# KDL-umass/CausalGPSLC.jl

Hardware: AMD Instinct MI355X
Metric: posterior samples/sec (kernel+chol+predict) at N=4096; SATE rel-err vs CPU (higher is better)
Workload: dtype f64; 1 GPU; Synthetic N=4096 D=8 nU=2, unit A (Gram build + potrf + alpha + MeanITE + SATE mean/var), L=1 level(s), 1024 posterior samples per GPU per step; levels=1, mean_ite=True

## Files before the change

### causalgpslc.jl_amd/csrc/k_gram.hip

```cpp
#include "gpslc_internal.h"
#include "gp_math.h"
#include <type_traits>

template <typename RT, int BIN, int FT>
__global__ __launch_bounds__(256) void gram_kernel(GramArgs g) {
    extern __shared__ __attribute__((aligned(16))) double sm[];
    const int F = FT > 0 ? FT : g.nU + g.nX;
    double* red = sm;
    double* etab = red + 4 * GP_TS * 2;
    RT* fr = reinterpret_cast<RT*>(etab + GP_EXP_TAB_DOUBLES);
    RT* fc = fr + F * GP_TS;
    RT* tr = fc + F * GP_TS;
    RT* tc = tr + GP_TS;

    const int tid = threadIdx.x;
    const int b = blockIdx.y;
    const long long s = g.s0 + b;
#ifdef GPSLC_DIAG
    const unsigned long long dt0 = g.dbg ? __builtin_amdgcn_s_memtime() : 0;
    const unsigned long long dr0 = g.dbg ? __builtin_amdgcn_s_memrealtime() : 0;
#endif
    int ti, tj;
    tri_decode(blockIdx.x, ti, tj);
    const int n = g.n;
    const int gi0 = ti * GP_TS, gj0 = tj * GP_TS;

    if (FT > 0) {
        constexpr int NIT = (FT * GP_TS + 255) / 256;
        constexpr bool CENTRE = std::is_same<RT, float>::value;
        double lv[NIT > 0 ? NIT : 1], av[NIT > 0 ? NIT : 1], cv[NIT > 0 ? NIT : 1];
        [[maybe_unused]] double x0[CENTRE && NIT > 0 ? NIT : 1];
#pragma unroll
        for (int k = 0; k < NIT; ++k) {
            const int idx = tid + 256 * k;
            const int f = min(idx >> 7, FT - 1), r = idx & 127;
            const double* src = g.column(s, f);
            lv[k] = g.lengthscale(s, f);
            av[k] = src[min(gi0 + r, n - 1)];
            cv[k] = src[min(gj0 + r, n - 1)];
            if constexpr (CENTRE) x0[k] = src[0];
        }
#pragma unroll
        for (int k = 0; k < NIT; ++k) {
            const int idx = tid + 256 * k;
            if (idx < FT * GP_TS) {
                const int f = idx >> 7, r = idx & 127;
                const double il = 1.0 / lv[k];
                if constexpr (CENTRE) { av[k] -= x0[k]; cv[k] -= x0[k]; }
                fr[f * GP_TS + r] = (RT)((gi0 + r < n) ? av[k] * il : 0.0);
                fc[f * GP_TS + r] = (RT)((gj0 + r < n) ? cv[k] * il : 0.0);
            }
        }
    } else {
        stage_scaled_features<GP_TS>(g, s, F, F, gi0, fr);
        stage_scaled_features<GP_TS>(g, s, F, F, gj0, fc);
    }
    if (tid < GP_TS) {
        tr[tid] = (RT)((gi0 + tid < n) ? centred_value<RT>(g.T, gi0 + tid) : 0.0);
        tc[tid] = (RT)((gj0 + tid < n) ? centred_value<RT>(g.T, gj0 + tid) : 0.0);
    }
    gp_exp_tab_stage(etab, tid);
    __syncthreads();
#ifdef GPSLC_DIAG
    const unsigned long long dt1 = g.dbg ? __builtin_amdgcn_s_memtime() : 0;
#endif

    const double ys = g.p.yScale[s];
    const double yn = g.p.yNoise[s];
    const double tl = g.p.tyLS[s];
    const RT wt = (RT)(1.0 / (tl * tl));
    const RT ew = RbfMath<RT>::exp_neg_t(-wt, etab);
    const int ty = tid & 15, tx = tid >> 4;

    RT tra[8];
#pragma unroll
    for (int p = 0; p < 8; ++p) tra[p] = tr[ty + 16 * p];

    double* tile = tref_tile(g.M, b, ti, tj);
    const int Np = g.nt * GP_TS;
    double* partB = g.part + ((long long)b * 2 + 0) * g.nt * Np;
    double* partK = g.part + ((long long)b * 2 + 1) * g.nt * Np;
    double rsB[8], rsK[8];
#pragma unroll
    for (int p = 0; p < 8; ++p) { rsB[p] = 0.0; rsK[p] = 0.0; }

    auto columns = [&](auto fast_tag) {
        constexpr bool FAST = decltype(fast_tag)::value;
#pragma unroll 1
        for (int q = 0; q < 8; ++q) {
            const int cq = 8 * tx + q;
            const int gj = gj0 + cq;
            RT lux[8];
#pragma unroll
            for (int p = 0; p < 8; ++p) lux[p] = (RT)0;
#pragma unroll 2
            for (int f = 0; f < (FT > 0 ? FT : F); ++f) {
                const RT c = fc[f * GP_TS + cq];
#pragma unroll
                for (int p = 0; p < 8; ++p) {
                    const RT d = fr[f * GP_TS + ty + 16 * p] - c;
                    lux[p] = fma(d, d, lux[p]);
                }
            }
            const RT tcq = tc[cq];
            double csB = 0.0, csK = 0.0;
#pragma unroll
            for (int p = 0; p < 8; ++p) {
                const int rp = ty + 16 * p;
                const int gi = gi0 + rp;
                const RT dt = tra[p] - tcq;
                const RT Bq = (RT)ys * RbfMath<RT>::exp_neg_t(-lux[p], etab);
                const RT Eq = BIN ? (dt == (RT)0 ? (RT)1 : ew) : RbfMath<RT>::exp_neg_t(-((dt * dt) * wt), etab);
                double Bv, Kv, Av;
                if (FAST) {
                    Bv = (double)Bq; Kv = (double)Bq * (double)Eq; Av = Kv;
                } else {
                    const bool inside = (gi < n) && (gj < n);
                    Bv = inside ? (double)Bq : 0.0;
                    Kv = inside ? (double)Bq * (double)Eq : 0.0;
                    Av = (gi == gj) ? (inside ? Kv + yn : 1.0) : Kv;
                }
                __builtin_nontemporal_store(Av, &tile[cq * GP_TS + rp]);
                rsB[p] += Bv; rsK[p] += Kv;
                csB += Bv; csK += Kv;
            }
            if (g.with_sums) {
#pragma unroll
                for (int o = 1; o <= 8; o <<= 1) { csB += __shfl_xor(csB, o, 64); csK += __shfl_xor(csK, o, 64); }
                if (ty == 0) {
                    partB[(long long)ti * Np + gj] = csB;
                    partK[(long long)ti * Np + gj] = csK;
                }
            }
        }
    };
    if (ti != tj && gi0 + GP_TS <= n && gj0 + GP_TS <= n) columns(std::true_type{});
    else columns(std::false_type{});
#ifdef GPSLC_DIAG
    if (g.dbg) {
        const unsigned long long dt2 = __builtin_amdgcn_s_memtime();
        asm volatile("s_waitcnt vmcnt(0)" ::: "memory");
        if (tid == 0) {
            unsigned long long* d = g.dbg + 8 * ((size_t)blockIdx.y * gridDim.x + blockIdx.x);
            d[0] = dt0; d[1] = dt1; d[2] = dt2; d[3] = __builtin_amdgcn_s_memtime();
            d[4] = dr0; d[5] = __builtin_amdgcn_s_memrealtime();
        }
    }
#endif
    if (!g.with_sums || ti == tj) return;

    const int wave = tid >> 6, lane = tid & 63;
    __syncthreads();
#pragma unroll
    for (int p = 0; p < 8; ++p) {
        double vb = rsB[p], vk = rsK[p];
        vb += __shfl_xor(vb, 16, 64); vk += __shfl_xor(vk, 16, 64);
        vb += __shfl_xor(vb, 32, 64); vk += __shfl_xor(vk, 32, 64);
        if (lane < 16) {
            red[(wave * GP_TS + ty + 16 * p) * 2 + 0] = vb;
            red[(wave * GP_TS + ty + 16 * p) * 2 + 1] = vk;
        }
    }
    __syncthreads();
    if (tid < GP_TS) {
        const double vb = (red[(0 * GP_TS + tid) * 2] + red[(1 * GP_TS + tid) * 2]) +
                          (red[(2 * GP_TS + tid) * 2] + red[(3 * GP_TS + tid) * 2]);
        const double vk = (red[(0 * GP_TS + tid) * 2 + 1] + red[(1 * GP_TS + tid) * 2 + 1]) +
                          (red[(2 * GP_TS + tid) * 2 + 1] + red[(3 * GP_TS + tid) * 2 + 1]);
        partB[(long long)tj * Np + gi0 + tid] = vb;
        partK[(long long)tj * Np + gi0 + tid] = vk;
    }
}

#define GRAM_LDS_BYTES(F, RTS) (4 * GP_TS * 2 * 8 + GP_EXP_TAB_DOUBLES * 8 + (2 * (F) * GP_TS + 2 * GP_TS) * (RTS))

template <typename RT, int BIN, int FT>
static void launch_gram_t(const GramArgs& g, int nbatch, hipStream_t st) {
    const int F = g.nU + g.nX;
    static DeviceOnce attr_set;
    lds_opt_in(attr_set, (const void*)gram_kernel<RT, BIN, FT>, GRAM_LDS_BYTES(MAXF, (int)sizeof(RT)));
    const int nlow = g.nt * (g.nt + 1) / 2;
    hipLaunchKernelGGL((gram_kernel<RT, BIN, FT>), dim3(nlow, nbatch), dim3(256), GRAM_LDS_BYTES(F, (int)sizeof(RT)), st, g);
}
template <typename RT, int BIN>
static void launch_gram_b(const GramArgs& g, int nbatch, hipStream_t st) {
    switch (g.nU + g.nX) {
        case 4: launch_gram_t<RT, BIN, 4>(g, nbatch, st); break;
        case 5: launch_gram_t<RT, BIN, 5>(g, nbatch, st); break;
        case 6: launch_gram_t<RT, BIN, 6>(g, nbatch, st); break;
        case 8: launch_gram_t<RT, BIN, 8>(g, nbatch, st); break;
        case 10: launch_gram_t<RT, BIN, 10>(g, nbatch, st); break;
        case 12: launch_gram_t<RT, BIN, 12>(g, nbatch, st); break;
        case 20: launch_gram_t<RT, BIN, 20>(g, nbatch, st); break;
        default: launch_gram_t<RT, BIN, 0>(g, nbatch, st); break;
    }
}
void launch_gram(const GramArgs& g, int nbatch, hipStream_t st) {
    if (g.f32) { if (g.binary_t) launch_gram_b<float, 1>(g, nbatch, st); else launch_gram_b<float, 0>(g, nbatch, st); }
    else { if (g.binary_t) launch_gram_b<double, 1>(g, nbatch, st); else launch_gram_b<double, 0>(g, nbatch, st); }
}

template <int FORM>
__global__ __launch_bounds__(256) void rhs_prepare_kernel(RhsArgs a) {
    using LF = LevelForm<FORM>;
    __shared__ double red[4];
    const int tid = threadIdx.x;
    const int b = blockIdx.x;
    const long long s = a.s0 + b;
    const int Np = a.nt * GP_TS;
    const double* partB = a.part + ((long long)b * 2 + 0) * a.nt * Np;
    const double* partK = a.part + ((long long)b * 2 + 1) * a.nt * Np;
    double* bs = a.bsum + (long long)b * Np;
    double* ks = a.ksum + (long long)b * Np;
    double tb = 0.0, tk = 0.0;
    for (int j = tid; j < Np; j += 256) {
        double vb = 0.0, vk = 0.0;
        for (int slot = 0; slot < a.nt; ++slot) {
            vb += partB[(long long)slot * Np + j];
            vk += partK[(long long)slot * Np + j];
        }
        bs[j] = vb; ks[j] = vk;
        tb += vb; tk += vk;
    }
    const double btot = block_sum_256(tb, red);
    const double ktot = block_sum_256(tk, red);
    const double tl = a.tyLS[s];
    const double wt = 1.0 / (tl * tl);
    const int L = a.lv.L;
    if constexpr (!LF::factual) {
        for (int l = tid; l < L; l += 256) {
            const double rho = LF::paired ? gp_rho(a.lv.doT[l], a.lv.base[l], wt) : 0.0;
            a.sumdelta[(long long)b * L + l] = LF::prior(rho, wt) * btot;
        }
        return;
    }
    for (int l = 0; l < L; ++l) {
        const double dot = a.lv.doT[l];
        double acc = 0.0;
        for (int j = tid; j < Np; j += 256) {
            const double r = gp_rho(j < a.n ? a.T[j] : 0.0, dot, wt);
            acc += r * bs[j];
        }
        const double rb = block_sum_256(acc, red);
        if (tid == 0) a.sumdelta[(long long)b * L + l] = (ktot - 2.0 * rb) + btot;
    }
}

template <int FORM>
__device__ __forceinline__ double rhs_level_value(const RhsArgs& a, int l, int gj, double wt, const double* bs, const double* ks) {
    using LF = LevelForm<FORM>;
    const double r = gp_rho(a.T[gj], a.lv.doT[l], wt);
    const double rb = LF::paired ? gp_rho(a.T[gj], a.lv.base[l], wt) : 0.0;
    const double x = LF::cross(a.T[gj] - a.lv.doT[l], r, rb, wt);
    if constexpr (LF::factual) return x * bs[gj] - ks[gj];
    else return x * bs[gj];
}
template <int FORM>
__global__ __launch_bounds__(256) void rhs_tiles_kernel(RhsArgs a) {
    const int tid = threadIdx.x;
    const int j = blockIdx.x, au = blockIdx.y, b = blockIdx.z;
    if (j > a.nt + au) return;
    const long long s = a.s0 + b;
    double* tile = tref_tile(a.M, b, a.nt + au, j);
    if (j >= a.nt) {
        if (a.live_rows > 0) return;
        for (int idx = tid; idx < GP_TSQ; idx += 256) tile[idx] = 0.0;
        return;
    }
    const int Np = a.nt * GP_TS;
    const int L = a.lv.L, R = L * a.G;
    const double tl = a.tyLS[s];
    const double wt = 1.0 / (tl * tl);
    const int sh = a.live_rows > 0 ? 5 : 7;
    for (int idx = tid; idx < (GP_TS << sh); idx += 256) {
        const int c = idx >> sh, q = idx & ((1 << sh) - 1);
        const int gq = au * GP_TS + q;
        const int gj = j * GP_TS + c;
        double v = 0.0;
        if (gj < a.n) {
            if (gq == 0) v = a.Y[s * a.y_sstride + gj];
            else if (gq <= R) {
                const int g = a.G > 1 ? (gq - 1) / L : 0, l = gq - 1 - L * g;
                const long long o = ((long long)b * a.G + g) * Np;
                v = rhs_level_value<FORM>(a, l, gj, wt, a.bw + o, a.kw + o);
            }
        }
        tile[c * GP_TS + q] = v;
    }
}

template <int FORM>
__global__ __launch_bounds__(256) void rhs_w_prepare_kernel(RhsArgs a) {
    using LF = LevelForm<FORM>;
    __shared__ double red[4];
    const int tid = threadIdx.x;
    const int qq = blockIdx.x, b = blockIdx.y;
    const int L = a.lv.L, l = qq % L, g = qq / L;
    const long long s = a.s0 + b;
    const int Np = a.nt * GP_TS;
    const double* bs = a.bw + ((long long)b * a.G + g) * Np;
    const double* ks = a.kw + ((long long)b * a.G + g) * Np;
    const double tl = a.tyLS[s];
    const double wt = 1.0 / (tl * tl);
    const double dot = a.lv.doT[l];
    double acc = 0.0, ww = 0.0;
    for (int j = tid; j < a.n; j += 256) {
        const double w = a.W[(long long)j * a.G + g];
        ww = fma(w, w, ww);
        if constexpr (!LF::factual) {
            acc += w * bs[j];
        } else {
            const double r = gp_rho(a.T[j], dot, wt);
            acc += w * ((ks[j] - 2.0 * r * bs[j]) + bs[j]);
        }
    }
    const double tot = block_sum_256(acc, red);
    if (l == 0) {
        const double w2 = block_sum_256(ww, red);
        if (tid == 0) a.wnorm2[(long long)b * a.G + g] = w2;
    }
    if (tid != 0) return;
    const double rho = LF::paired ? gp_rho(dot, a.lv.base[l], wt) : 0.0;
    if constexpr (LF::factual) a.sumdelta[(long long)b * L * a.G + qq] = tot;
    else a.sumdelta[(long long)b * L * a.G + qq] = LF::prior(rho, wt) * tot;
}

template <int FORM>
static void launch_rhs_t(const RhsArgs& r, int nbatch, hipStream_t st, bool sums_given) {
    if (r.W && !sums_given) hipLaunchKernelGGL(rhs_w_prepare_kernel<FORM>, dim3(r.lv.L * r.G, nbatch), dim3(256), 0, st, r);
    else if (r.with_sums && !sums_given) hipLaunchKernelGGL(rhs_prepare_kernel<FORM>, dim3(nbatch), dim3(256), 0, st, r);
    hipLaunchKernelGGL(rhs_tiles_kernel<FORM>, dim3(r.nt + r.naug, r.naug, nbatch), dim3(256), 0, st, r);
}
void launch_rhs(const RhsArgs& r, int nbatch, hipStream_t st, bool sums_given) {
    dispatch_form(r.lv.form, [&](auto form) { launch_rhs_t<decltype(form)::value>(r, nbatch, st, sums_given); });
}

__global__ __launch_bounds__(256) void epilogue_kernel(EpiArgs e) {
    __shared__ double red[4];
    const int tid = threadIdx.x;
    const int b = blockIdx.x;
    const long long s = e.s0 + b;
    double acc = 0.0;
    for (int i = tid; i < e.n; i += 256) {
        const int k = i >> 7, c = i & 127;
        const double* dt = tref_tile(e.M, b, k, k);
        acc += log(dt[c * GP_TS + c]);
    }
    const double ld = 2.0 * block_sum_256(acc, red);
    const double nn = (double)e.n;
    auto put_level = [&](int l, double zw, double ww) {
        const double sd = e.sumdelta[(long long)b * e.L + l];
        if (e.wnorm2) {
            if (e.meanSATE) e.meanSATE[s + e.S * l] = zw;
            if (e.varSATE) e.varSATE[s + e.S * l] = (sd - ww) + e.pred_noise * e.wnorm2[(long long)b * (e.L / e.wL) + l / e.wL];
            return;
        }
        if (e.meanSATE) e.meanSATE[s + e.S * l] = zw / nn;
        if (e.varSATE) e.varSATE[s + e.S * l] = ((sd - ww) + nn * e.pred_noise) / (nn * nn);
    };
    if (e.from_rows) {
        const int lane = tid & 63, wave = tid >> 6;
        const int ncol = e.nt * GP_TS;
        const int nq = (e.meanSATE || e.varSATE) ? e.L : 0;
        if (tid == 0 && e.logdet) e.logdet[s] = ld;
        auto put = [&](int q, double zw, double ww) {
            if (q == 0) { if (e.quad) e.quad[s] = ww; return; }
            put_level(q - 1, zw, ww);
        };
        if (nq >= 16) {
            for (int qb = 16 * wave; qb <= nq; qb += 64) {
                double zw[16], ww[16];
#pragma unroll
                for (int j = 0; j < 16; ++j) { zw[j] = 0.0; ww[j] = 0.0; }
                for (int i = lane; i < ncol; i += 64) {
                    const double* col = tref_tile(e.M, b, e.nt, i >> 7) + (long long)(i & 127) * GP_TS;
                    const double z = col[0];
#pragma unroll
                    for (int j = 0; j < 16; ++j) {
                        const double w = col[qb + j];
                        zw[j] = fma(z, w, zw[j]);
                        ww[j] = fma(w, w, ww[j]);
                    }
                }
#pragma unroll
                for (int j = 0; j < 16; ++j) {
                    double a = zw[j], c = ww[j];
#pragma unroll
                    for (int o = 32; o >= 1; o >>= 1) { a += __shfl_xor(a, o, 64); c += __shfl_xor(c, o, 64); }
                    if (lane == 0 && qb + j <= nq) put(qb + j, a, c);
                }
            }
            return;
        }
        for (int q = wave; q <= nq; q += 4) {
            double zw = 0.0, ww = 0.0;
            for (int i = lane; i < ncol; i += 64) {
                const double* col = tref_tile(e.M, b, e.nt, i >> 7) + (long long)(i & 127) * GP_TS;
                const double z = col[0], w = col[q];
                zw = fma(z, w, zw);
                ww = fma(w, w, ww);
            }
#pragma unroll
            for (int o = 32; o >= 1; o >>= 1) { zw += __shfl_xor(zw, o, 64); ww += __shfl_xor(ww, o, 64); }
            if (lane == 0) put(q, zw, ww);
        }
        return;
    }
    const double* g00 = tref_tile(e.M, b, e.nt, e.nt);
    if (tid == 0) {
        if (e.logdet) e.logdet[s] = ld;
        if (e.quad) e.quad[s] = -g00[0];
    }
    if (e.meanSATE == nullptr && e.varSATE == nullptr) return;
    for (int l = tid; l < e.L; l += 256) {
        const int q = 1 + l, au = q >> 7, qq = q & 127;
        const double wz = -tref_tile(e.M, b, e.nt + au, e.nt)[0 * GP_TS + qq];
        const double ww = -tref_tile(e.M, b, e.nt + au, e.nt + au)[qq * GP_TS + qq];
        put_level(l, wz, ww);
    }
}

void launch_epilogue(const EpiArgs& e, int nbatch, hipStream_t st) {
    hipLaunchKernelGGL(epilogue_kernel, dim3(nbatch), dim3(256), 0, st, e);
}

__global__ __launch_bounds__(256) void rbf_log_kernel(const double* X1, const double* X2, long long n,
                                                      int d, const double* ls, int ls_len, double* out) {
    const long long i = (long long)blockIdx.x * 16 + (threadIdx.x & 15);
    const long long ip = (long long)blockIdx.y * 16 + (threadIdx.x >> 4);
    if (i >= n || ip >= n) return;
    double acc = 0.0;
    for (int k = 0; k < d; ++k) {
        const double l = ls[ls_len == 1 ? 0 : k];
        const double df = X1[i + n * k] - X2[ip + n * k];
        acc += (df * df) / (l * l);
    }
    out[i + n * ip] = -acc;
}

void launch_rbf_log(const double* X1, const double* X2, long long n, int d, const double* ls,
                    int ls_len, double* out, hipStream_t st) {
    dim3 grid((unsigned)((n + 15) / 16), (unsigned)((n + 15) / 16));
    hipLaunchKernelGGL(rbf_log_kernel, grid, dim3(256), 0, st, X1, X2, n, d, ls, ls_len, out);
}

__global__ __launch_bounds__(256) void process_cov_kernel(const double* in, long long n, double scale,
                                                          double noise, double* out) {
    const long long idx = (long long)blockIdx.x * 256 + threadIdx.x;
    if (idx >= n * n) return;
    const long long i = idx % n, j = idx / n;
    double v = exp(in[idx]) * scale;
    if (i == j) v += noise;
    out[idx] = v;
}

void launch_process_cov(const double* in, long long n, double scale, double noise, double* out,
                        hipStream_t st) {
    const long long tot = n * n;
    hipLaunchKernelGGL(process_cov_kernel, dim3((unsigned)((tot + 255) / 256)), dim3(256), 0, st, in, n,
                       scale, noise, out);
}

__global__ __launch_bounds__(256) void dense_load_kernel(DenseLoadArgs a) {
    int ti, tj;
    tri_decode(blockIdx.x, ti, tj);
    double* tile = tref_tile(a.M, 0, ti, tj);
    for (int idx = threadIdx.x; idx < GP_TSQ; idx += 256) {
        const int c = idx >> 7, r = idx & 127;
        const long long gi = (long long)ti * GP_TS + r, gj = (long long)tj * GP_TS + c;
        double v;
        if (gi < a.n && gj < a.n) v = a.cov[gi + (long long)a.n * gj];
        else v = (gi == gj) ? 1.0 : 0.0;
        tile[idx] = v;
    }
}
void launch_dense_load(const DenseLoadArgs& a, hipStream_t st) {
    hipLaunchKernelGGL(dense_load_kernel, dim3(a.nt * (a.nt + 1) / 2), dim3(256), 0, st, a);
}

__global__ __launch_bounds__(256) void rows_rhs_kernel(RowsRhsArgs a) {
    const int j = blockIdx.x, au = blockIdx.y;
    if (a.rect ? (j >= a.nt) : (j > a.nt + au)) return;
    double* tile = tref_tile(a.M, 0, a.row0 + au, j);
    for (int idx = threadIdx.x; idx < GP_TSQ; idx += 256) {
        const int c = idx >> 7, q = idx & 127;
        const long long gq = (long long)au * GP_TS + q, gj = (long long)j * GP_TS + c;
        double v = 0.0;
        if (j < a.nt && gq < a.S && gj < a.n) v = a.x[gj + (long long)a.n * gq];
        tile[idx] = v;
    }
}
void launch_rows_rhs(const RowsRhsArgs& a, hipStream_t st) {
    hipLaunchKernelGGL(rows_rhs_kernel, dim3(a.nt + a.naug, a.naug), dim3(256), 0, st, a);
}

__global__ __launch_bounds__(256) void quad_rows_kernel(QuadRowsArgs a) {
    __shared__ double red[4];
    const int tid = threadIdx.x;
    double acc = 0.0;
    for (int i = tid; i < a.n; i += 256) {
        const double* dt = tref_tile(a.M, 0, i >> 7, i >> 7);
        acc += log(dt[(i & 127) * GP_TS + (i & 127)]);
    }
    const double ld = 2.0 * block_sum_256(acc, red);
    if (tid == 0) a.logdet[0] = ld;
    for (long long q = tid; q < a.S; q += 256) {
        const int au = (int)(q >> 7), qq = (int)(q & 127);
        a.quad[q] = -tref_tile(a.M, 0, a.nt + au, a.nt + au)[qq * GP_TS + qq];
    }
}
__global__ __launch_bounds__(128) void row_norms_kernel(RowNormArgs a) {
    const int au = blockIdx.x, q = threadIdx.x;
    double acc = 0.0;
    for (int j = 0; j < a.nt; ++j) {
        const double* t = tref_tile(a.W, 0, au, j);
        for (int c = 0; c < GP_TS; ++c) {
            const double v = t[c * GP_TS + q];
            acc = fma(v, v, acc);
        }
    }
    const long long gq = (long long)au * GP_TS + q;
    if (gq < a.S) a.quad[gq] = acc;
}
void launch_row_norms(const RowNormArgs& a, hipStream_t st) {
    hipLaunchKernelGGL(row_norms_kernel, dim3(a.naug), dim3(128), 0, st, a);
}

void launch_quad_rows(const QuadRowsArgs& a, hipStream_t st) {
    hipLaunchKernelGGL(quad_rows_kernel, dim3(1), dim3(256), 0, st, a);
}
```

### causalgpslc.jl_amd/csrc/k_solve.hip

```cpp
#include "gpslc_internal.h"
#include "gp_math.h"
#include "back_block.h"
#include "pair_mfma.h"
#include <stdexcept>

__global__ __launch_bounds__(256) void backsolve_alpha_kernel(BackArgs a, int i, double* alpha) {
    __shared__ double zi[GP_TS];
    const int tid = threadIdx.x, lane = tid & 63, wave = tid >> 6;
    const long long b = blockIdx.x;
    const int Np = a.nt * GP_TS;
    if (tid < GP_TS) zi[tid] = a.zwork[b * Np + i * GP_TS + tid];
    __syncthreads();
    const double* invt = a.inv + b * a.inv_bstride + (long long)i * GP_TSQ;
    double o32[32];
    tile_tv32(invt, zi, wave, lane, o32);
    if (lane == 0) {
#pragma unroll
        for (int cc = 0; cc < 32; ++cc) alpha[b * Np + i * GP_TS + wave * 32 + cc] = o32[cc];
    }
}
__global__ __launch_bounds__(256) void backsolve_update_kernel(BackArgs a, int i, const double* alpha) {
    __shared__ double ai[GP_TS];
    const int tid = threadIdx.x, lane = tid & 63, wave = tid >> 6;
    const int k = blockIdx.x;
    const long long b = blockIdx.y;
    const int Np = a.nt * GP_TS;
    if (tid < GP_TS) ai[tid] = alpha[b * Np + i * GP_TS + tid];
    __syncthreads();
    double o32[32];
    tile_tv32(tref_tile(a.M, b, i, k), ai, wave, lane, o32);
    double* z = a.zwork + b * Np;
    if (lane == 0) {
#pragma unroll
        for (int cc = 0; cc < 32; ++cc) z[k * GP_TS + wave * 32 + cc] -= o32[cc];
    }
}

__global__ __launch_bounds__(128) void extract_z_kernel(BackArgs a) {
    const int j = blockIdx.x;
    const long long b = blockIdx.y;
    const double* t = tref_tile(a.M, b, a.nt, j);
    a.zwork[b * a.nt * GP_TS + j * GP_TS + threadIdx.x] = t[threadIdx.x * GP_TS + 0];
}

void launch_backsolve(const BackArgs& a, int nbatch, hipStream_t st) {
    double* alpha = a.zwork + (long long)nbatch * a.nt * GP_TS;
    hipLaunchKernelGGL(extract_z_kernel, dim3(a.nt, nbatch), dim3(128), 0, st, a);
    for (int i = a.nt - 1; i >= 0; --i) {
        hipLaunchKernelGGL(backsolve_alpha_kernel, dim3(nbatch), dim3(256), 0, st, a, i, alpha);
        if (i > 0) hipLaunchKernelGGL(backsolve_update_kernel, dim3(i, nbatch), dim3(256), 0, st, a, i, alpha);
    }
}

template <int FREG, int LCT, typename RT, int RB, int FORM = FORM_ORDINARY>
__global__ __launch_bounds__(256) void ite_mean_kernel(IteMeanArgs a) {
    using LF = LevelForm<FORM>;
    extern __shared__ __attribute__((aligned(16))) double sm[];
    const int F = a.nU + a.nX;
    double* etab = sm;
    double* rl = etab + GP_EXP_TAB_DOUBLES;
    double* red = rl + LCT * GP_TS;
    RT* fc = reinterpret_cast<RT*>(red + RB * GP_TS * LCT);
    const int tid = threadIdx.x, r = tid & 127, h = tid >> 7;
    const int ib = blockIdx.x;
    const long long b = blockIdx.y, s = a.s0 + b;
    const int n = a.n, Np = a.nt * GP_TS;

    auto feat_src = [&](int f) { return a.column(s, f); };
    auto feat_il = [&](int f) { return 1.0 / a.lengthscale(s, f); };
    int gi[RB];
    RT af[RB][FREG];
#pragma unroll
    for (int q = 0; q < RB; ++q) {
        gi[q] = (ib * RB + q) * GP_TS + r;
#pragma unroll
        for (int f = 0; f < FREG; ++f) af[q][f] = (RT)((f < F && gi[q] < n) ? centred_value<RT>(feat_src(f), gi[q]) * feat_il(f) : 0.0);
    }
    const double ys = a.p.yScale[s];
    const double tl = a.p.tyLS[s];
    const double wt = 1.0 / (tl * tl);
    const RT wtq = (RT)wt;
    gp_exp_tab_stage(etab, tid);
    const double* alpha = a.alpha + b * Np;

    const int L = a.lv.L;
    const double* doT = a.lv.doT;
    for (int l0 = 0; l0 < L; l0 += LCT) {
        const int nl = min(LCT, L - l0);
        double acc[RB][LCT];
#pragma unroll
        for (int q = 0; q < RB; ++q)
#pragma unroll
            for (int ll = 0; ll < LCT; ++ll) acc[q][ll] = 0.0;
        for (int jt = 0; jt < a.nt; ++jt) {
            __syncthreads();
            stage_scaled_features<GP_TS>(a, s, F, FREG, jt * GP_TS, fc);
            for (int idx = tid; idx < LCT * GP_TS; idx += 256) {
                const int ll = idx >> 7, cc = idx & 127;
                const int g = jt * GP_TS + cc;
                double v = 0.0;
                if (ll < nl && g < n) {
                    const double dt64 = a.T[g] - doT[l0 + ll];
                    const RT dt = (RT)dt64, db = LF::paired ? (RT)(a.T[g] - a.lv.base[l0 + ll]) : (RT)0;
                    const double rb = LF::paired ? (double)RbfMath<RT>::exp_neg_t(-((db * db) * wtq), etab) : 0.0;
                    v = LF::cross(dt64, (double)RbfMath<RT>::exp_neg_t(-((dt * dt) * wtq), etab), rb, wt) * alpha[g];
                }
                rl[idx] = v;
            }
            __syncthreads();
#pragma unroll 2
            for (int cq = 0; cq < 64; ++cq) {
                const int c = h * 64 + cq;
                RT cf[FREG];
#pragma unroll
                for (int f = 0; f < FREG; ++f) cf[f] = fc[f * GP_TS + c];
                double rlc[LCT];
#pragma unroll
                for (int ll = 0; ll < LCT; ++ll) rlc[ll] = rl[ll * GP_TS + c];
#pragma unroll
                for (int q = 0; q < RB; ++q) {
                    RT lux = (RT)0;
#pragma unroll
                    for (int f = 0; f < FREG; ++f) {
                        const RT d = af[q][f] - cf[f];
                        lux = fma(d, d, lux);
                    }
                    const double Bv = (double)((RT)ys * RbfMath<RT>::exp_neg_t(-lux, etab));
#pragma unroll
                    for (int ll = 0; ll < LCT; ++ll) acc[q][ll] = fma(Bv, rlc[ll], acc[q][ll]);
                }
            }
        }
        __syncthreads();
        if (h == 1) {
#pragma unroll
            for (int q = 0; q < RB; ++q)
#pragma unroll
                for (int ll = 0; ll < LCT; ++ll) red[(q * GP_TS + r) * LCT + ll] = acc[q][ll];
        }
        __syncthreads();
        if (h == 0) {
#pragma unroll
            for (int q = 0; q < RB; ++q) {
                if (gi[q] >= n) continue;
                if constexpr (!LF::factual) {
#pragma unroll
                    for (int ll = 0; ll < LCT; ++ll)
                        if (ll < nl) {
                            const double v = acc[q][ll] + red[(q * GP_TS + r) * LCT + ll];
                            a.meanITE[(long long)gi[q] * a.si + s * a.ss + (long long)(l0 + ll) * a.sl] =
                                (LF::paired && LF::zero_level(doT[l0 + ll], a.lv.base[l0 + ll])) ? 0.0 : v;
                        }
                    continue;
                }
                const double ka = a.Y[s * a.y_sstride + gi[q]] - a.yNoise[s] * alpha[gi[q]];
                const double ti = a.T[gi[q]];
#pragma unroll
                for (int ll = 0; ll < LCT; ++ll)
                    if (ll < nl) {
                        const double v = (acc[q][ll] + red[(q * GP_TS + r) * LCT + ll]) - ka;
                        a.meanITE[(long long)gi[q] * a.si + s * a.ss + (long long)(l0 + ll) * a.sl] =
                            (ti == doT[l0 + ll]) ? 0.0 : v;
                    }
            }
        }
    }
}

template <int FREG, int FORM = FORM_ORDINARY>
__global__ __launch_bounds__(256, 2) void ite_mean_mfma_kernel(IteMeanArgs a) {
    extern __shared__ __attribute__((aligned(16))) double sm[];
    const long long b = blockIdx.y, s = a.s0 + b;
    const double* alpha = a.alpha + b * (a.nt * GP_TS);
    using LF = LevelForm<FORM>;
    const double* doT = a.lv.doT;
    pair_mfma_body<FREG, false, 0>(
        a, s, a.lv.L, sm,
        [&](int j, int l, double wt, const double* etab) {
            const double dt = a.T[j] - doT[l], db = LF::paired ? a.T[j] - a.lv.base[l] : 0.0;
            const double rb = LF::paired ? gp_exp_neg_tab(-((db * db) * wt), etab) : 0.0;
            return LF::cross(dt, gp_exp_neg_tab(-((dt * dt) * wt), etab), rb, wt) * alpha[j];
        },
        [&](int gi, int l0, int nl, const d4* acc, const d4*) {
            if (gi >= a.n) return;
            double* out = a.meanITE + (long long)gi * a.si + s * a.ss;
            if constexpr (!LF::factual) {
                pair_mfma_each_column(nl, [&](int q, int v, int ll) {
                    out[(long long)(l0 + ll) * a.sl] = (LF::paired && LF::zero_level(doT[l0 + ll], a.lv.base[l0 + ll])) ? 0.0 : acc[q][v];
                });
                return;
            }
            const double ka = a.Y[s * a.y_sstride + gi] - a.yNoise[s] * alpha[gi];
            const double ti = a.T[gi];
            pair_mfma_each_column(nl, [&](int q, int v, int ll) {
                out[(long long)(l0 + ll) * a.sl] = (ti == doT[l0 + ll]) ? 0.0 : acc[q][v] - ka;
            });
        });
}

template <int FORM>
static void launch_ite_mean_mfma(const IteMeanArgs& a, int nbatch, hipStream_t st) {
    pair_mfma_freg_ladder(a.nU + a.nX, [&](auto freg) {
        constexpr int FREG = decltype(freg)::value;
        pair_mfma_launch<ite_mean_mfma_kernel<FREG, FORM>, FREG, false>(a, nbatch, st);
    });
}

template <int FREG, int LCT, typename RT, int FORM>
static void launch_ite_mean_t(const IteMeanArgs& a, int nbatch, hipStream_t st) {
    constexpr int RB = 1;
    const int bytes = (GP_EXP_TAB_DOUBLES + (1 + RB) * LCT * GP_TS) * 8 + (FREG * GP_TS) * (int)sizeof(RT);
    static DeviceOnce attr_set;
    lds_opt_in(attr_set, (const void*)ite_mean_kernel<FREG, LCT, RT, RB, FORM>, bytes);
    hipLaunchKernelGGL((ite_mean_kernel<FREG, LCT, RT, RB, FORM>), dim3((a.nt + RB - 1) / RB, nbatch), dim3(256), bytes, st, a);
}
template <int FREG, typename RT, int FORM>
static void launch_ite_mean_f(const IteMeanArgs& a, int nbatch, hipStream_t st) {
    if (a.lv.L <= 1) launch_ite_mean_t<FREG, 1, RT, FORM>(a, nbatch, st);
    else if (a.lv.L <= 4) launch_ite_mean_t<FREG, 4, RT, FORM>(a, nbatch, st);
    else if constexpr (LevelForm<FORM>::fp32_kernels) launch_ite_mean_t<FREG, 16, RT, FORM>(a, nbatch, st);
}
template <typename RT, int FORM>
static void launch_ite_mean_r(const IteMeanArgs& a, int nbatch, hipStream_t st) {
    const int F = a.nU + a.nX;
    if (F <= 4) launch_ite_mean_f<4, RT, FORM>(a, nbatch, st);
    else if (F <= 5) launch_ite_mean_f<5, RT, FORM>(a, nbatch, st);
    else if (F <= 6) launch_ite_mean_f<6, RT, FORM>(a, nbatch, st);
    else if (F <= 8) launch_ite_mean_f<8, RT, FORM>(a, nbatch, st);
    else if (F <= 10) launch_ite_mean_f<10, RT, FORM>(a, nbatch, st);
    else if (F <= 12) launch_ite_mean_f<12, RT, FORM>(a, nbatch, st);
    else if (F <= 16) launch_ite_mean_f<16, RT, FORM>(a, nbatch, st);
    else if (F <= 20) launch_ite_mean_f<20, RT, FORM>(a, nbatch, st);
    else launch_ite_mean_f<32, RT, FORM>(a, nbatch, st);
}
void launch_ite_mean(const IteMeanArgs& a, int nbatch, hipStream_t st) {
    dispatch_form(a.lv.form, [&](auto form) {
        constexpr int FORM = decltype(form)::value;
        if constexpr (LevelForm<FORM>::fp32_kernels) {
            if (a.f32) { launch_ite_mean_r<float, FORM>(a, nbatch, st); return; }
        }
        if (a.lv.L > 4) launch_ite_mean_mfma<FORM>(a, nbatch, st);
        else launch_ite_mean_r<double, FORM>(a, nbatch, st);
    });
}

enum { LEVEL_NONE, LEVEL_SCALAR, LEVEL_VECTOR, LEVEL_VECTOR_OUTCOME };
struct LevelTerms { double e, gij, gji, h; };
template <bool VEC>
__device__ __forceinline__ LevelTerms level_terms(double ti, double tj, double xi, double xj, double wt) {
    const double e = gp_rho(ti, tj, wt);
    if (VEC) return {e, gp_rho(ti, xj, wt), gp_rho(tj, xi, wt), gp_rho(xi, xj, wt)};
    return {e, xi, xj, 1.0};
}
__device__ __forceinline__ LevelTerms level_terms_outcome(double tj, double xi, double xj, double wt) {
    return {0.0, 0.0, gp_rho(tj, xi, wt), gp_rho(xi, xj, wt)};
}
constexpr int tile_build_lds_bytes(int F) { return (2 * F * GP_TS + 4 * GP_TS) * 8; }

template <int LEVEL, typename StageLevel, typename Emit>
__device__ __forceinline__ void tile_build_body(const SampleGrid& a, long long s, int ti, int tj, double* sm,
                                                StageLevel&& stage_level, Emit&& emit) {
    const int F = a.nU + a.nX;
    double* fr = sm;
    double* fc = fr + F * GP_TS;
    double* tr = fc + F * GP_TS;
    double* tc = tr + GP_TS;
    double* rr_ = tc + GP_TS;
    double* rc_ = rr_ + GP_TS;
    const int tid = threadIdx.x;
    const int n = a.n;
    const int gi0 = ti * GP_TS, gj0 = tj * GP_TS;
    const double tl = a.p.tyLS[s];
    const double wt = 1.0 / (tl * tl);
    stage_scaled_features<GP_TS>(a, s, F, F, gi0, fr);
    stage_scaled_features<GP_TS>(a, s, F, F, gj0, fc);
    if (tid < GP_TS) {
        const double t1 = (gi0 + tid < n) ? a.T[gi0 + tid] : 0.0;
        const double t2 = (gj0 + tid < n) ? a.T[gj0 + tid] : 0.0;
        tr[tid] = t1; tc[tid] = t2;
        if (LEVEL != LEVEL_NONE) rr_[tid] = stage_level(gi0 + tid, t1, wt);
        rc_[tid] = stage_level(gj0 + tid, t2, wt);
    }
    __syncthreads();
    const double ys = a.p.yScale[s];
    const int ty = tid & 15, tx = tid >> 4;
#pragma unroll 1
    for (int q = 0; q < 8; ++q) {
        const int cq = 8 * tx + q;
        const int gj = gj0 + cq;
        double lux[8];
#pragma unroll
        for (int p = 0; p < 8; ++p) lux[p] = 0.0;
        for (int f = 0; f < F; ++f) {
            const double c = fc[f * GP_TS + cq];
#pragma unroll
            for (int p = 0; p < 8; ++p) {
                const double d = fr[f * GP_TS + ty + 16 * p] - c;
                lux[p] = fma(d, d, lux[p]);
            }
        }
        const double tcq = tc[cq], xj = rc_[cq];
#pragma unroll
        for (int p = 0; p < 8; ++p) {
            const int rp = ty + 16 * p;
            const int gi = gi0 + rp;
            const bool inside = (gi < n) && (gj < n);
            double Bv = 0.0;
            LevelTerms t{0.0, 0.0, xj, 0.0};
            if (LEVEL == LEVEL_NONE || inside) {
                Bv = ys * gp_exp_neg(-lux[p]);
                if constexpr (LEVEL == LEVEL_VECTOR_OUTCOME) t = level_terms_outcome(tcq, rr_[rp], xj, wt);
                else if constexpr (LEVEL != LEVEL_NONE) t = level_terms<LEVEL == LEVEL_VECTOR>(tr[rp], tcq, rr_[rp], xj, wt);
            }
            emit(rp, cq, inside, gi == gj, Bv, t);
        }
    }
}

template <bool VEC, int FORM = FORM_ORDINARY>
__global__ __launch_bounds__(256) void dt_build_kernel(DtArgs a) {
    using LF = LevelForm<FORM>;
    constexpr bool NOLV = !LF::factual && !VEC;
    extern __shared__ __attribute__((aligned(16))) double sm[];
    const int ti = blockIdx.x / a.nt, tj = blockIdx.x % a.nt;
    const long long b = blockIdx.y, s = a.s0 + b / a.lc;
    const int l = a.l0 + (int)(b % a.lc), n = a.n;
    const double doT = VEC ? 0.0 : a.lv.doT[l], doTb = LF::paired ? a.lv.base[l] : 0.0;
    const double* dv = VEC ? a.lv.doT + (long long)n * l : nullptr;
    double kss = 0.0;
    if constexpr (NOLV) {
        const double tl = a.p.tyLS[s];
        const double wt = 1.0 / (tl * tl);
        kss = LF::prior(LF::paired ? gp_rho(doT, doTb, wt) : 0.0, wt);
    }
    double* wt_tile = tref_tile(a.W, b, ti, tj);
    double* c_tile = (ti >= tj) ? tref_tile(a.Cm, b, ti, tj) : nullptr;
    tile_build_body<NOLV ? LEVEL_NONE : !VEC ? LEVEL_SCALAR : LF::factual ? LEVEL_VECTOR : LEVEL_VECTOR_OUTCOME>(
        a, s, ti, tj, sm,
        [&](int g, double t, double wt) {
            if constexpr (VEC) return g < n ? dv[g] : 0.0;
            else return LF::cross(t - doT, gp_rho(t, doT, wt), LF::paired ? gp_rho(t, doTb, wt) : 0.0, wt);
        },
        [&](int rp, int cq, bool inside, bool diag, double Bv, const LevelTerms& t) {
            double Dv, Cv;
            if constexpr (!LF::factual) {
                Dv = Bv * t.gji;
                Cv = VEC ? Bv * t.h : Bv * kss;
            } else {
                Dv = Bv * (t.gji - t.e);
                Cv = Bv * (((t.e - t.gij) - t.gji) + t.h);
            }
            if (!inside) { Dv = 0.0; Cv = diag ? 1.0 : 0.0; }
            else if (diag) Cv += a.pred_noise;
            wt_tile[cq * GP_TS + rp] = Dv;
            if (c_tile) c_tile[cq * GP_TS + rp] = Cv;
        });
}

template <bool VEC, int FORM = FORM_ORDINARY>
static void launch_dt_build_t(const DtArgs& a, int nbatch, hipStream_t st) {
    static DeviceOnce attr_set;
    lds_opt_in(attr_set, (const void*)dt_build_kernel<VEC, FORM>, tile_build_lds_bytes(MAXF));
    hipLaunchKernelGGL((dt_build_kernel<VEC, FORM>), dim3(a.nt * a.nt, nbatch), dim3(256), tile_build_lds_bytes(a.nU + a.nX), st, a);
}
void launch_dt_build(const DtArgs& a, int nbatch, hipStream_t st) {
    dispatch_form(a.lv.form, [&](auto form) {
        constexpr int FORM = decltype(form)::value;
        if (!a.lv.vec) launch_dt_build_t<false, FORM>(a, nbatch, st);
        else if constexpr (LevelForm<FORM>::vector_levels) launch_dt_build_t<true, FORM>(a, nbatch, st);
        else throw std::logic_error("this level form has no vector-level kernels");
    });
}

__global__ __launch_bounds__(256) void gather_cov_kernel(GatherCovArgs a) {
    int ti, tj;
    tri_decode(blockIdx.x, ti, tj);
    const long long b = blockIdx.y, s = a.s0 + b;
    const double* t = tref_tile(a.Cm, b, ti, tj);
    for (int idx = threadIdx.x; idx < GP_TSQ; idx += 256) {
        const int c = idx >> 7, r = idx & 127;
        const long long gi = (long long)ti * GP_TS + r, gj = (long long)tj * GP_TS + c;
        if (gi >= a.n || gj >= a.n || gi < gj) continue;
        const double v = t[idx];
        a.out[s + a.S * (gi + a.n * gj)] = v;
        a.out[s + a.S * (gj + a.n * gi)] = v;
    }
}
void launch_gather_cov(const GatherCovArgs& a, int nbatch, hipStream_t st) {
    hipLaunchKernelGGL(gather_cov_kernel, dim3(a.nt * (a.nt + 1) / 2, nbatch), dim3(256), 0, st, a);
}

template <bool VEC>
__global__ __launch_bounds__(256) void ld_build_kernel(LdBuildArgs a) {
    extern __shared__ __attribute__((aligned(16))) double sm[];
    const int ti = blockIdx.x / a.nt, tj = blockIdx.x % a.nt;
    const int n = a.n;
    double* tK = tref_tile(a.K, 0, ti, tj);
    double* tKs = tref_tile(a.Ks, 0, ti, tj);
    double* tKsT = tref_tile(a.KsT, 0, ti, tj);
    double* tKss = tref_tile(a.Kss, 0, ti, tj);
    tile_build_body<VEC ? LEVEL_VECTOR : LEVEL_SCALAR>(
        a, a.s0, ti, tj, sm,
        [&](int g, double t, double wt) {
            if constexpr (VEC) return g < n ? a.doTv[g] : 0.0;
            else return gp_rho(t, a.doT, wt);
        },
        [&](int rp, int cq, bool inside, bool, double Bv, const LevelTerms& t) {
            const int idx = cq * GP_TS + rp;
            tK[idx] = inside ? Bv * t.e : 0.0;
            tKs[idx] = inside ? t.gij * Bv : 0.0;
            tKsT[idx] = inside ? Bv * t.gji : 0.0;
            tKss[idx] = inside ? Bv * t.h : 0.0;
        });
}
template <bool VEC>
static void launch_ld_build_t(const LdBuildArgs& a, hipStream_t st) {
    static DeviceOnce attr_set;
    lds_opt_in(attr_set, (const void*)ld_build_kernel<VEC>, tile_build_lds_bytes(MAXF));
    hipLaunchKernelGGL(ld_build_kernel<VEC>, dim3(a.nt * a.nt), dim3(256), tile_build_lds_bytes(a.nU + a.nX), st, a);
}
void launch_ld_build(const LdBuildArgs& a, hipStream_t st) {
    if (a.doTv) launch_ld_build_t<true>(a, st);
    else launch_ld_build_t<false>(a, st);
}

__global__ __launch_bounds__(256) void rect_gather_kernel(RectGatherArgs a) {
    const int ti = blockIdx.x / a.nt, tj = blockIdx.x % a.nt;
    const double* t = tref_tile(a.R, 0, ti, tj);
    for (int idx = threadIdx.x; idx < GP_TSQ; idx += 256) {
        const int c = idx >> 7, r = idx & 127;
        const long long gi = (long long)ti * GP_TS + r, gj = (long long)tj * GP_TS + c;
        if (gi < a.n && gj < a.n) a.out[gi + (long long)a.n * gj] = t[idx] + (gi == gj ? a.diag_add : 0.0);
    }
}
void launch_rect_gather(const RectGatherArgs& a, hipStream_t st) {
    hipLaunchKernelGGL(rect_gather_kernel, dim3(a.nt * a.nt), dim3(256), 0, st, a);
}

__device__ __forceinline__ double julia_quantile_sorted(const double* v, int m, double p) {
#pragma clang fp contract(off)
    if (m == 1) return v[0];
    const double aleph = (double)m * p + (1.0 - p);
    int j = (int)aleph;
    j = min(max(j, 1), m - 1);
    double gam = aleph - (double)j;
    gam = fmin(fmax(gam, 0.0), 1.0);
    const double a = v[j - 1], b = v[j];
    return a + gam * (b - a);
}

__global__ __launch_bounds__(256) void summarize_kernel(SummArgs a) {
    extern __shared__ __attribute__((aligned(16))) double v[];
    __shared__ double red[4];
    const int tid = threadIdx.x;
    const long long i = blockIdx.x;
    double acc = 0.0;
    for (int j = tid; j < a.mpad; j += 256) {
        double x = INFINITY;
        if (j < a.m) { x = a.x[i * a.rs + (long long)j * a.cs]; acc += x; }
        v[j] = x;
    }
#pragma unroll
    for (int o = 32; o >= 1; o >>= 1) acc += __shfl_xor(acc, o, 64);
    if ((tid & 63) == 0) red[tid >> 6] = acc;
    __syncthreads();
    const double total = (red[0] + red[1]) + (red[2] + red[3]);
    for (int k = 2; k <= a.mpad; k <<= 1) {
        for (int j = k >> 1; j > 0; j >>= 1) {
            for (int t = tid; t < a.mpad; t += 256) {
                const int u = t ^ j;
                if (u > t) {
                    const bool up = (t & k) == 0;
                    const double p = v[t], q = v[u];
                    if ((p > q) == up) { v[t] = q; v[u] = p; }
                }
            }
            __syncthreads();
        }
    }
    if (tid == 0) {
        a.mean[i] = total / (double)a.m;
        a.lower[i] = julia_quantile_sorted(v, a.m, a.lowerQ);
        a.upper[i] = julia_quantile_sorted(v, a.m, a.upperQ);
    }
}
#define SUMM_RW 16
__device__ __forceinline__ unsigned long long summ_key(double x) {
    const unsigned long long b = (unsigned long long)__double_as_longlong(x);
    return (b >> 63) ? ~b : (b | 0x8000000000000000ull);
}
__device__ __forceinline__ double summ_unkey(unsigned long long k) {
    const unsigned long long b = (k >> 63) ? (k & 0x7fffffffffffffffull) : ~k;
    return __longlong_as_double((long long)b);
}
__global__ __launch_bounds__(256) void summarize_select_kernel(SummArgs a) {
    __shared__ unsigned int hist[SUMM_RW][2][256];
    __shared__ unsigned long long prefix[SUMM_RW][2], mingt[SUMM_RW][2];
    __shared__ unsigned int rank[SUMM_RW][2], cntle[SUMM_RW][2];
    __shared__ double rsum[4][SUMM_RW];
    const int tid = threadIdx.x, r = tid & (SUMM_RW - 1), jj = tid >> 4;
    const long long i = (long long)blockIdx.x * SUMM_RW + r;
    const bool live = i < a.n;
    const double* row = a.x + (live ? i : 0) * a.rs;
    const int m = a.m;
    int jq[2];
    double gq[2];
    {
#pragma clang fp contract(off)
        const double ps[2] = {a.lowerQ, a.upperQ};
        for (int q = 0; q < 2; ++q) {
            const double aleph = (double)m * ps[q] + (1.0 - ps[q]);
            int j = (int)aleph;
            j = min(max(j, 1), m - 1);
            jq[q] = j;
            gq[q] = fmin(fmax(aleph - (double)j, 0.0), 1.0);
        }
    }
    for (int t = tid; t < SUMM_RW * 2 * 256; t += 256) (&hist[0][0][0])[t] = 0u;
    if (tid < SUMM_RW * 2) {
        const int rr = tid & (SUMM_RW - 1), q = tid >> 4;
        prefix[rr][q] = 0ull; rank[rr][q] = (unsigned)(jq[q] - 1); cntle[rr][q] = 0u; mingt[rr][q] = ~0ull;
    }
    double acc = 0.0;
    if (live)
        for (int j = jj; j < m; j += 16) acc += row[(long long)j * a.cs];
    acc += __shfl_xor(acc, 16, 64);
    acc += __shfl_xor(acc, 32, 64);
    if ((tid & 63) < SUMM_RW) rsum[tid >> 6][r] = acc;
    __syncthreads();
    for (int pass = 0; pass < 8; ++pass) {
        const int shift = 56 - 8 * pass;
        if (live) {
            const unsigned long long p0 = prefix[r][0], p1 = prefix[r][1];
            for (int j = jj; j < m; j += 16) {
                const unsigned long long k = summ_key(row[(long long)j * a.cs]);
                const unsigned long long hi = pass == 0 ? 0ull : (k >> (shift + 8));
                const unsigned d = (unsigned)(k >> shift) & 255u;
                if (hi == p0) atomicAdd(&hist[r][0][d], 1u);
                if (hi == p1) atomicAdd(&hist[r][1][d], 1u);
            }
        }
        __syncthreads();
        if (tid < SUMM_RW * 2) {
            const int rr = tid & (SUMM_RW - 1), q = tid >> 4;
            unsigned cum = 0, want = rank[rr][q], d = 0;
            for (; d < 255u; ++d) {
                const unsigned cnt = hist[rr][q][d];
                if (want < cum + cnt) break;
                cum += cnt;
            }
            prefix[rr][q] = (prefix[rr][q] << 8) | d;
            rank[rr][q] = want - cum;
        }
        __syncthreads();
        for (int t = tid; t < SUMM_RW * 2 * 256; t += 256) (&hist[0][0][0])[t] = 0u;
        __syncthreads();
    }
    if (live) {
        const unsigned long long k0 = prefix[r][0], k1 = prefix[r][1];
        unsigned c0 = 0, c1 = 0;
        unsigned long long g0 = ~0ull, g1 = ~0ull;
        for (int j = jj; j < m; j += 16) {
            const unsigned long long k = summ_key(row[(long long)j * a.cs]);
            if (k <= k0) ++c0; else g0 = k < g0 ? k : g0;
            if (k <= k1) ++c1; else g1 = k < g1 ? k : g1;
        }
        atomicAdd(&cntle[r][0], c0); atomicAdd(&cntle[r][1], c1);
        atomicMin(&mingt[r][0], g0); atomicMin(&mingt[r][1], g1);
    }
    __syncthreads();
    if (tid < SUMM_RW && i < a.n) {
#pragma clang fp contract(off)
        double qv[2];
        for (int q = 0; q < 2; ++q) {
            const double av = summ_unkey(prefix[r][q]);
            const double bv = cntle[r][q] > (unsigned)jq[q] ? av : summ_unkey(mingt[r][q]);
            qv[q] = m == 1 ? av : av + gq[q] * (bv - av);
        }
        a.mean[i] = ((rsum[0][r] + rsum[1][r]) + (rsum[2][r] + rsum[3][r])) / (double)m;
        a.lower[i] = qv[0];
        a.upper[i] = qv[1];
    }
}

void launch_summarize(const SummArgs& a, hipStream_t st) {
    if (a.m > 16384) {
        hipLaunchKernelGGL(summarize_select_kernel, dim3((a.n + SUMM_RW - 1) / SUMM_RW), dim3(256), 0, st, a);
        return;
    }
    static DeviceOnce attr_set;
    lds_opt_in(attr_set, (const void*)summarize_kernel, 16384 * 8);
    hipLaunchKernelGGL(summarize_kernel, dim3(a.n), dim3(256), (size_t)a.mpad * 8, st, a);
}
```

Before: 2467 posterior samples/s.

## Register-block gram columns and restage ITE-mean features with cached scales

The Gram kernel now computes squared distances for two columns at once. It reuses each loaded row-feature value across both columns, adds scheduling barriers, and pins the sum accumulation order so contraction is disabled. The ITE-mean kernel replaces the generic feature-staging helper with an inline staging loop. That loop caches inverse lengthscales, centring offsets and level values in LDS and batches global loads per thread, and the per-tile barrier moves to the end of the loop. This cuts redundant LDS reads and per-element lengthscale recomputation, at the cost of more registers and a slightly larger shared-memory footprint.

```diff
diff --git a/causalgpslc.jl_amd/csrc/k_gram.hip b/causalgpslc.jl_amd/csrc/k_gram.hip
--- a/causalgpslc.jl_amd/csrc/k_gram.hip
+++ b/causalgpslc.jl_amd/csrc/k_gram.hip
@@ -84,24 +84,11 @@
 #pragma unroll
     for (int p = 0; p < 8; ++p) { rsB[p] = 0.0; rsK[p] = 0.0; }
 
+    constexpr int QW = 2;
     auto columns = [&](auto fast_tag) {
         constexpr bool FAST = decltype(fast_tag)::value;
-#pragma unroll 1
-        for (int q = 0; q < 8; ++q) {
-            const int cq = 8 * tx + q;
+        auto column = [&](int cq, const RT* lux) {
             const int gj = gj0 + cq;
-            RT lux[8];
-#pragma unroll
-            for (int p = 0; p < 8; ++p) lux[p] = (RT)0;
-#pragma unroll 2
-            for (int f = 0; f < (FT > 0 ? FT : F); ++f) {
-                const RT c = fc[f * GP_TS + cq];
-#pragma unroll
-                for (int p = 0; p < 8; ++p) {
-                    const RT d = fr[f * GP_TS + ty + 16 * p] - c;
-                    lux[p] = fma(d, d, lux[p]);
-                }
-            }
             const RT tcq = tc[cq];
             double csB = 0.0, csK = 0.0;
 #pragma unroll
@@ -121,8 +108,12 @@
                     Av = (gi == gj) ? (inside ? Kv + yn : 1.0) : Kv;
                 }
                 __builtin_nontemporal_store(Av, &tile[cq * GP_TS + rp]);
-                rsB[p] += Bv; rsK[p] += Kv;
-                csB += Bv; csK += Kv;
+                {
+#pragma clang fp contract(off)
+                    rsB[p] += Bv; rsK[p] += Kv;
+                    csB += Bv; csK += Kv;
+                }
+                asm volatile("" : "+v"(rsB[p]), "+v"(rsK[p]), "+v"(csB), "+v"(csK));
             }
             if (g.with_sums) {
 #pragma unroll
@@ -132,6 +123,34 @@
                     partK[(long long)ti * Np + gj] = csK;
                 }
             }
+        };
+#pragma unroll 1
+        for (int q0 = 0; q0 < 8; q0 += QW) {
+            const int cq0 = 8 * tx + q0;
+            RT lux[QW][8];
+#pragma unroll
+            for (int w = 0; w < QW; ++w)
+#pragma unroll
+                for (int p = 0; p < 8; ++p) lux[w][p] = (RT)0;
+#pragma unroll 1
+            for (int f = 0; f < (FT > 0 ? FT : F); ++f) {
+                RT c[QW], av[8];
+#pragma unroll
+                for (int w = 0; w < QW; ++w) c[w] = fc[f * GP_TS + cq0 + w];
+#pragma unroll
+                for (int p = 0; p < 8; ++p) av[p] = fr[f * GP_TS + ty + 16 * p];
+#pragma unroll
+                for (int p = 0; p < 8; ++p) {
+                    if (p % 2 == 0 && p) __builtin_amdgcn_sched_barrier(0x104);
+#pragma unroll
+                    for (int w = 0; w < QW; ++w) {
+                        const RT d = av[p] - c[w];
+                        lux[w][p] = fma(d, d, lux[w][p]);
+                    }
+                }
+            }
+#pragma unroll
+            for (int w = 0; w < QW; ++w) column(cq0 + w, lux[w]);
         }
     };
     if (ti != tj && gi0 + GP_TS <= n && gj0 + GP_TS <= n) columns(std::true_type{});
diff --git a/causalgpslc.jl_amd/csrc/k_solve.hip b/causalgpslc.jl_amd/csrc/k_solve.hip
--- a/causalgpslc.jl_amd/csrc/k_solve.hip
+++ b/causalgpslc.jl_amd/csrc/k_solve.hip
@@ -58,7 +58,11 @@
     extern __shared__ __attribute__((aligned(16))) double sm[];
     const int F = a.nU + a.nX;
     double* etab = sm;
-    double* rl = etab + GP_EXP_TAB_DOUBLES;
+    double* ils = etab + GP_EXP_TAB_DOUBLES;
+    double* x0s = ils + FREG;
+    double* dts = x0s + FREG;
+    double* bss = dts + LCT;
+    double* rl = bss + LCT;
     double* red = rl + LCT * GP_TS;
     RT* fc = reinterpret_cast<RT*>(red + RB * GP_TS * LCT);
     const int tid = threadIdx.x, r = tid & 127, h = tid >> 7;
@@ -81,7 +85,44 @@
     const double wt = 1.0 / (tl * tl);
     const RT wtq = (RT)wt;
     gp_exp_tab_stage(etab, tid);
+    if (tid < FREG) {
+        ils[tid] = tid < F ? feat_il(tid) : 0.0;
+        x0s[tid] = (std::is_same<RT, float>::value && tid < F) ? feat_src(tid)[0] : 0.0;
+    }
     const double* alpha = a.alpha + b * Np;
+
+    constexpr int NIT = (FREG * GP_TS + 255) / 256;
+    constexpr int KCH = NIT <= 6 ? NIT : 4;
+    auto stage = [&](int jt, int nl) {
+        const int g = jt * GP_TS + r, gc = min(g, n - 1);
+        const double tg = a.T[gc], ag = alpha[gc];
+#pragma unroll 1
+        for (int k0 = 0; k0 < NIT; k0 += KCH) {
+            double x[KCH];
+#pragma unroll
+            for (int k = 0; k < KCH; ++k) {
+                const int f = h + 2 * (k0 + k);
+                x[k] = (f < F ? feat_src(f) : a.T)[gc];
+            }
+#pragma unroll
+            for (int k = 0; k < KCH; ++k) {
+                const int f = h + 2 * (k0 + k);
+                if (f < FREG) fc[f * GP_TS + r] = (RT)((f < F && g < n) ? (std::is_same<RT, float>::value ? x[k] - x0s[f] : x[k]) * ils[f] : 0.0);
+            }
+        }
+#pragma unroll 1
+        for (int idx = tid; idx < LCT * GP_TS; idx += 256) {
+            const int ll = idx >> 7;
+            double v = 0.0;
+            if (ll < nl && g < n) {
+                const double dt64 = tg - dts[ll];
+                const RT dt = (RT)dt64, db = LF::paired ? (RT)(tg - bss[ll]) : (RT)0;
+                const double rb = LF::paired ? (double)RbfMath<RT>::exp_neg_t(-((db * db) * wtq), etab) : 0.0;
+                v = LF::cross(dt64, (double)RbfMath<RT>::exp_neg_t(-((dt * dt) * wtq), etab), rb, wt) * ag;
+            }
+            rl[idx] = v;
+        }
+    };
 
     const int L = a.lv.L;
     const double* doT = a.lv.doT;
@@ -92,21 +133,14 @@
         for (int q = 0; q < RB; ++q)
 #pragma unroll
             for (int ll = 0; ll < LCT; ++ll) acc[q][ll] = 0.0;
+        __syncthreads();
+        if (tid < nl) {
+            dts[tid] = doT[l0 + tid];
+            if (LF::paired) bss[tid] = a.lv.base[l0 + tid];
+        }
+        __syncthreads();
         for (int jt = 0; jt < a.nt; ++jt) {
-            __syncthreads();
-            stage_scaled_features<GP_TS>(a, s, F, FREG, jt * GP_TS, fc);
-            for (int idx = tid; idx < LCT * GP_TS; idx += 256) {
-                const int ll = idx >> 7, cc = idx & 127;
-                const int g = jt * GP_TS + cc;
-                double v = 0.0;
-                if (ll < nl && g < n) {
-                    const double dt64 = a.T[g] - doT[l0 + ll];
-                    const RT dt = (RT)dt64, db = LF::paired ? (RT)(a.T[g] - a.lv.base[l0 + ll]) : (RT)0;
-                    const double rb = LF::paired ? (double)RbfMath<RT>::exp_neg_t(-((db * db) * wtq), etab) : 0.0;
-                    v = LF::cross(dt64, (double)RbfMath<RT>::exp_neg_t(-((dt * dt) * wtq), etab), rb, wt) * alpha[g];
-                }
-                rl[idx] = v;
-            }
+            stage(jt, nl);
             __syncthreads();
 #pragma unroll 2
             for (int cq = 0; cq < 64; ++cq) {
@@ -130,8 +164,8 @@
                     for (int ll = 0; ll < LCT; ++ll) acc[q][ll] = fma(Bv, rlc[ll], acc[q][ll]);
                 }
             }
-        }
-        __syncthreads();
+            __syncthreads();
+        }
         if (h == 1) {
 #pragma unroll
             for (int q = 0; q < RB; ++q)
@@ -209,7 +243,7 @@
 template <int FREG, int LCT, typename RT, int FORM>
 static void launch_ite_mean_t(const IteMeanArgs& a, int nbatch, hipStream_t st) {
     constexpr int RB = 1;
-    const int bytes = (GP_EXP_TAB_DOUBLES + (1 + RB) * LCT * GP_TS) * 8 + (FREG * GP_TS) * (int)sizeof(RT);
+    const int bytes = (GP_EXP_TAB_DOUBLES + 2 * FREG + 2 * LCT + (1 + RB) * LCT * GP_TS) * 8 + (FREG * GP_TS) * (int)sizeof(RT);
     static DeviceOnce attr_set;
     lds_opt_in(attr_set, (const void*)ite_mean_kernel<FREG, LCT, RT, RB, FORM>, bytes);
     hipLaunchKernelGGL((ite_mean_kernel<FREG, LCT, RT, RB, FORM>), dim3((a.nt + RB - 1) / RB, nbatch), dim3(256), bytes, st, a);
```

Result: no change. 2479 posterior samples/s, median of 6 (+0.5%).
